# Bergvca/string_grouper

Hardware: AMD Instinct MI355X
Metric: hot-path rows/sec (the device path of match_strings: tokenise + tf-idf + postings + SpGEMM-topn, inputs resident in HBM), 663k-name self-join ntop=10 min_sim=0.8; match_strings end to end: match_strings_rows_per_s (higher is better)
Workload: dtype f32

## Files before the change

### string_grouper_amd/csrc/sg_internal.h

```cpp
#pragma once

#include <hip/hip_runtime.h>
#include <stdint.h>
#include <stdio.h>
#include <stdlib.h>
#include <string.h>

#include <map>
#include <memory>
#include <mutex>
#include <new>
#include <string>
#include <vector>

#include "../../include/sg_hip.h"

#define SG_WAVE 64
#define SG_NUM_XCD 8

void sg_set_error(const char *fmt, ...);

#define SG_HIP_TRY(expr)                                                                        \
    do {                                                                                        \
        hipError_t _e = (expr);                                                                 \
// ... 164 lines not shown
struct sg_csr {
    sg_ctx *ctx = nullptr;
    int64_t n_rows = 0, n_cols = 0, nnz = 0;
    int32_t dtype = SG_F32;
    const int64_t *d_indptr = nullptr;
    const int32_t *d_indices = nullptr;
    const void *d_data = nullptr;
    bool owned = false;
    mutable int props_state = 0;
    mutable float props_max_norm2 = 0.f;
    mutable uint32_t props_max_nnz = 0;
    bool from_vectoriser = false;
    mutable bool props_by_construction = false;
    mutable bool props_repeated_column = false;
    uint32_t *d_props_words = nullptr;
    double *d_row_norm = nullptr;
    mutable int left_state = 0;
    mutable struct SgCollapse *left_groups = nullptr;
    struct SgCollapse *rows_of = nullptr;
};

struct SgScoreCtx {
    const uint32_t *fwd_ptr = nullptr;
    const void *fwd = nullptr;
    const uint32_t *orig_of = nullptr;
    const void *blk = nullptr;
    uint32_t blk_bytes = 0;
    const uint4 *q8 = nullptr;
    float q8_scale = 0.f;
    uint32_t pad_ = 0;
};
#define SG_Q8_STRIDE 256u
#define SG_Q8_MAX_ENTRIES 60u

struct SgCollapse {
    sg_ctx *ctx = nullptr;
    int64_t n_orig = 0, n_u = 0;
    uint32_t *d_gid = nullptr;
    uint32_t *d_group_ptr = nullptr;
    uint32_t *d_members = nullptr;
    uint32_t *d_rep_rows = nullptr;
    int64_t *d_rep_start = nullptr;
    int32_t *d_rep_len = nullptr;
    struct sg_csr *unique = nullptr;
    const struct sg_csr *pending_src = nullptr;
};

struct sg_postings {
    sg_ctx *ctx = nullptr;
    int64_t n_right = 0, n_terms = 0, nnz = 0;
    int32_t dtype = SG_F32;
    int32_t tile_log2 = 12;
    int32_t n_tiles = 0;
    const int64_t *b_indptr = nullptr;
    const int32_t *b_indices = nullptr;
    const void *b_data = nullptr;
    uint32_t *d_seg = nullptr;
    uint32_t *d_term_len = nullptr;
    uint32_t *d_term_start = nullptr;
    int32_t *d_rows = nullptr;
    void *d_vals = nullptr;
    sg_csr src;
    int32_t split = 1;
    void *d_fwd = nullptr;
    uint32_t *d_fwd_ptr = nullptr;
    void *d_blk = nullptr;
    uint32_t blk_bytes = 0;
    void *d_q8 = nullptr;
    uint32_t *d_filt = nullptr;
    sg_csr *permuted = nullptr;
    uint32_t *d_orig_of = nullptr, *d_pos_of = nullptr;
    struct SgScoreCtx *d_score_ctx = nullptr;
    uint32_t *d_ends = nullptr;
    int32_t nt_pad = 0;
    int32_t fold_log2 = 0;
    uint32_t *d_ends8 = nullptr;
    int32_t nv_pad = 0;
    float norm_up = 0.f;
    uint32_t freq_min = 0;
    bool cosine_like = false;
    float max_norm2 = 0.f;
    SgCollapse *collapse = nullptr;
    const sg_csr *caller_b = nullptr;
    sg_csr caller_b_copy;
    int64_t n_right_caller = 0;
    mutable sg_postings *plain = nullptr;
    mutable sg_postings *exact_native = nullptr;
    mutable sg_postings *alt_tile = nullptr;
    sg_csr built_from;
    bool built_from_valid = false;
    bool tile_form = false;
    const sg_postings *view_of = nullptr;
    int32_t build_tile_cols = 0, build_flags = 0;
};

struct sg_topn {
    sg_ctx *ctx = nullptr;
    int64_t n_rows = 0, n_cols = 0;
    int32_t stride = 0;
    int32_t dtype = SG_F32;
    int32_t top_n_asked = 0;
// ... 6 lines not shown
    void operator()(sg_topn *r) const { sg_topn_free(r); }
};
using TopnPtr = std::unique_ptr<sg_topn, TopnFree>;
int topn_alloc(sg_ctx *ctx, int64_t n_rows, int64_t n_cols, int32_t stride, int32_t dtype, TopnPtr *out);
bool result_stride(int64_t n_rows, int64_t top_n, int64_t n_cols, int32_t *stride);
int result_overflow(int64_t n_rows, int32_t stride, const char *advice);
int sort_rows_by_column(sg_ctx *ctx, sg_topn *r);

struct sg_vocab {
    sg_ctx *ctx = nullptr;
    sg_vec_params params;
    int32_t bits_per_char = 7;
    int64_t n_terms = 0, n_docs = 0;
    int64_t key_space = 0;
    bool sorted_mode = false;
    int32_t *d_key_to_col = nullptr;
    uint64_t *d_keys = nullptr;
    int32_t *d_df = nullptr;
    void *d_idf = nullptr;
    bool idf_trusted = false;
    struct VocabImpl *impl = nullptr;
};

int sg_matchlist_device_view(const sg_matchlist *ml, int64_t *n_rows, int64_t *n_cols, int64_t *n_entries, int32_t *dtype,
                             const int64_t **row_ptr, const int32_t **cols, const void **vals);

#define SG_POSTINGS_NO_COLLAPSE (1 << 8)
#define SG_POSTINGS_TILE_FORM (1 << 11)
#define SG_POSTINGS_EXACT_ONLY (1 << 10)
int sg_csr_props(sg_ctx *ctx, const sg_csr *m, bool *cosine_like, float *max_norm2, uint32_t *max_nnz = nullptr);
bool sg_pruned_supports_tile(int32_t tile_log2);
int sg_postings_ensure_full(sg_ctx *ctx, const sg_postings *p);
bool sg_q8_applies(const sg_ctx *ctx, const sg_postings *Bt, double threshold);
int sg_spgemm_pruned_launch(sg_ctx *ctx, const sg_csr *A, const sg_postings *Bt, int32_t keep, sg_topn *r,
                            double threshold, double delta, uint32_t *row_counter,
                            uint32_t *flagged_count, uint32_t *flagged_rows, unsigned long long *stats);

int sg_spgemm_pruned_symmetric(sg_ctx *ctx, const sg_csr *A, const sg_postings *Bt, int32_t keep, sg_topn *r,
                               double threshold, double delta, unsigned long long *stats, bool *done, int64_t row_lo = 0,
                               int64_t row_hi = -1 , int32_t **export_pairs = nullptr,
                               int64_t *export_n = nullptr, int64_t row_step = 1 ,
                               bool exact_all = false );
int sg_selfjoin_merge_pairs(sg_ctx *ctx, sg_topn *r, const int32_t *d_pairs, int64_t n_pairs, int64_t row_lo, int64_t row_hi,
                            const uint32_t *pos_of ,
                            int64_t row_step = 1);

#define SG_PAIR_CHUNK 256u
#define SG_PAIR_NO_CHUNK 0xFFFFFFFFu
struct SgPairSink {
    uint32_t *d_i = nullptr;
    uint32_t *d_j = nullptr;
    void *d_s = nullptr;
    uint32_t *d_row_count = nullptr;
    uint32_t *d_chunk_count = nullptr;
    uint32_t *d_chunks_used = nullptr;
    unsigned long long *d_totals = nullptr;
    uint32_t chunks = 0;
};
unsigned sg_spgemm_exact_selfjoin_grid(const sg_ctx *ctx, const sg_postings *Bt = nullptr );
int sg_spgemm_exact_selfjoin_rows(sg_ctx *ctx, const sg_csr *A, const sg_postings *Bt, int32_t keep, sg_topn *r,
                                  double threshold, uint32_t *row_counter, const uint32_t *row_list,
                                  const uint32_t *row_list_len, const SgPairSink &sink, bool all_rows = false);

int sg_collapse_build(sg_ctx *ctx, const sg_csr *B, SgCollapse **out, bool left_side = false, bool defer_rows = false);
int sg_collapse_materialize(sg_ctx *ctx, SgCollapse *c);
int sg_csr_ensure_rows(sg_ctx *ctx, const sg_csr *m);
// ... 15 lines not shown
```

### string_grouper_amd/csrc/sg_postings.hip

```cpp
#include <stdlib.h>

#include <memory>
#include <optional>

#include "sg_internal.h"
#include "sg_scan.h"

__device__ __forceinline__ int64_t row_of_thread(int64_t g, int32_t tile_log2, int32_t n_tiles) {
    return ((g % n_tiles) << tile_log2) | (g / n_tiles);
}

template <typename T>
__global__ void __launch_bounds__(256) postings_count(const int64_t *__restrict__ indptr,
                                                      const int32_t *__restrict__ indices, int64_t n_rows,
                                                      int32_t tile_log2, int32_t n_tiles, uint32_t *seg_counts) {
    const int64_t j = row_of_thread((int64_t)blockIdx.x * blockDim.x + threadIdx.x, tile_log2, n_tiles);
    if (j >= n_rows) return;
    const int64_t lo = indptr[j], hi = indptr[j + 1];
    const uint32_t t = (uint32_t)(j >> tile_log2);
    for (int64_t p = lo; p < hi; ++p) {
        const int64_t bin = (int64_t)indices[p] * n_tiles + t;
        atomicAdd(&seg_counts[bin], 1u);
    }
}
// ... 625 lines not shown
    if (ends8)
        for (int32_t v = 0; v < nv_pad; ++v) {
            int64_t t = (int64_t)(v + 1) << fold_log2;
            if (t > n_tiles) t = n_tiles;
            ends8[k * nv_pad + v] = k == n_terms ? 0u : seg[k * n_tiles + t] << 2;
        }
}

__global__ void __launch_bounds__(256) null_postings_kernel(uint32_t *__restrict__ slack) {
    const uint32_t i = blockIdx.x * blockDim.x + threadIdx.x;
    slack[i] = sg_null_posting(i);
}

struct PermutedLenLoad {
    uint64_t n, minv, magic;
    const int32_t *len_of_row;
    const int64_t *indptr;
    uint32_t *pos_of, *orig_of;
    __device__ __forceinline__ int64_t operator()(int64_t p) const {
        const uint64_t x = (uint64_t)p * minv;
        const uint64_t q = __umul64hi(x, magic);
        int64_t rem = (int64_t)(x - q * n);
        if (rem < 0) rem += (int64_t)n;
        const uint32_t g = (uint32_t)rem;
        orig_of[p] = g;
        pos_of[g] = (uint32_t)p;
        return len_of_row ? (int64_t)len_of_row[g] : indptr[g + 1] - indptr[g];
    }
};

__device__ __forceinline__ uint32_t sg_q8_units(int64_t nnz) {
    return nnz > (int64_t)SG_Q8_MAX_ENTRIES ? 1u : (uint32_t)((nnz + 7) >> 2);
}
template <typename T>
__device__ __forceinline__ void q8_write_unit(uint4 *__restrict__ rec, uint32_t u, const int32_t *__restrict__ indices,
                                              const T *__restrict__ data, int64_t src, int64_t nnz, uint32_t first_packed,
                                              uint32_t name, float inv_norm) {
    auto entry = [&](int64_t e) -> uint32_t {
        if (e >= nnz) return 0u;
        const float q = ceilf((float)data[src + e] * inv_norm * 255.0f * 1.000002f);
        const uint32_t bq = q >= 255.0f ? 255u : (q >= 1.0f ? (uint32_t)q : 1u);
        return ((uint32_t)indices[src + e] << 8) | bq;
    };
    uint4 w;
    if (u == 0) {
        w = make_uint4(first_packed, name, (uint32_t)nnz | (nnz <= (int64_t)SG_Q8_MAX_ENTRIES ? 0u : 0x80000000u), 0u);
    } else {
        const int64_t e0 = 4 * (int64_t)u - 4;
        w = make_uint4(entry(e0), entry(e0 + 1), entry(e0 + 2), entry(e0 + 3));
    }
    rec[u] = w;
}

template <typename T>
__global__ void __launch_bounds__(256) q8_pack_kernel(const int64_t *__restrict__ indptr, const int32_t *__restrict__ indices,
                                                      const T *__restrict__ data, int64_t n_rows,
                                                      const uint32_t *__restrict__ orig_of ,
                                                      uint4 *__restrict__ q8, float inv_norm) {
    const int64_t p = ((int64_t)blockIdx.x * blockDim.x + threadIdx.x) >> 4;
    const uint32_t sub = threadIdx.x & 15;
    if (p >= n_rows) return;
    const int64_t base = indptr[0], src = indptr[p], n = indptr[p + 1] - src;
    if (sub < sg_q8_units(n))
        q8_write_unit<T>(q8 + p * (SG_Q8_STRIDE / 16), sub, indices, data, src, n, (uint32_t)(src - base),
                         orig_of ? orig_of[p] : (uint32_t)p, inv_norm);
}

#ifndef SG_GATHER_ROWS
#define SG_GATHER_ROWS 2
#endif
template <typename T>
__device__ __forceinline__ uint32_t q8_entry_of(int32_t k, T v, bool have, float inv_norm) {
    if (!have) return 0u;
    const float q = ceilf((float)v * inv_norm * 255.0f * 1.000002f);
    const uint32_t bq = q >= 255.0f ? 255u : (q >= 1.0f ? (uint32_t)q : 1u);
    return ((uint32_t)k << 8) | bq;
}
__device__ __forceinline__ void q8_write_round(uint4 *__restrict__ rec, int r, uint32_t wq, int sub, uint32_t units) {
    const int q = (sub - 4 * r - 1) & 3;
    const int base = (int)(threadIdx.x & 48u) + 4 * q;
    const uint32_t x0 = (uint32_t)__shfl((int)wq, base, 64), x1 = (uint32_t)__shfl((int)wq, base + 1, 64);
    const uint32_t x2 = (uint32_t)__shfl((int)wq, base + 2, 64), x3 = (uint32_t)__shfl((int)wq, base + 3, 64);
    if (sub >= 4 * r + 1 && sub <= 4 * r + 4 && (uint32_t)sub < units) rec[sub] = make_uint4(x0, x1, x2, x3);
}
template <typename T>
__device__ __forceinline__ void store_packed(void *__restrict__ fwd, int64_t at, int32_t k, T v) {
    if (sizeof(T) == 4) {
        reinterpret_cast<int2 *>(fwd)[at] = make_int2(k, __float_as_int((float)v));
    } else {
        const long long bits = __double_as_longlong((double)v);
        reinterpret_cast<int4 *>(fwd)[at] = make_int4(k, 0, (int)(bits & 0xffffffffll), (int)(bits >> 32));
    }
}
template <typename T>
__global__ void __launch_bounds__(256) gather_rows_kernel(const int64_t *__restrict__ indptr, const int32_t *__restrict__ indices,
                                                          const T *__restrict__ data, int64_t n_rows,
                                                          const uint32_t *__restrict__ orig_of,
                                                          const uint32_t *__restrict__ rep_rows ,
                                                          const int64_t *__restrict__ rep_start ,
                                                          const int32_t *__restrict__ rep_len,
                                                          const int64_t *__restrict__ perm_ptr, int32_t *__restrict__ perm_indices,
                                                          T *__restrict__ perm_data,
                                                          uint32_t *__restrict__ fwd_ptr , void *__restrict__ fwd,
                                                          uint4 *__restrict__ q8 , float inv_norm) {
    const int64_t grp = ((int64_t)blockIdx.x * blockDim.x + threadIdx.x) >> 4;
    const int sub = threadIdx.x & 15;
    const int64_t p0 = grp * SG_GATHER_ROWS;
    if (p0 > n_rows) return;
    bool valid[SG_GATHER_ROWS];
    uint32_t g[SG_GATHER_ROWS];
    int64_t src[SG_GATHER_ROWS], dst[SG_GATHER_ROWS];
    int32_t n[SG_GATHER_ROWS];
#pragma unroll
    for (int i = 0; i < SG_GATHER_ROWS; ++i) {
        valid[i] = p0 + i < n_rows;
        g[i] = valid[i] ? orig_of[p0 + i] : 0u;
        dst[i] = p0 + i <= n_rows ? perm_ptr[p0 + i] : 0;
    }
    if (rep_start) {
#pragma unroll
        for (int i = 0; i < SG_GATHER_ROWS; ++i) {
            src[i] = valid[i] ? rep_start[g[i]] : 0;
            n[i] = valid[i] ? rep_len[g[i]] : 0;
        }
    } else {
        int64_t j[SG_GATHER_ROWS];
#pragma unroll
        for (int i = 0; i < SG_GATHER_ROWS; ++i) j[i] = (valid[i] && rep_rows) ? (int64_t)rep_rows[g[i]] : (int64_t)g[i];
#pragma unroll
        for (int i = 0; i < SG_GATHER_ROWS; ++i) {
            src[i] = valid[i] ? indptr[j[i]] : 0;
            n[i] = valid[i] ? (int32_t)(indptr[j[i] + 1] - src[i]) : 0;
        }
    }
    int32_t k[SG_GATHER_ROWS][2];
    T v[SG_GATHER_ROWS][2];
#pragma unroll
    for (int i = 0; i < SG_GATHER_ROWS; ++i)
#pragma unroll
        for (int r = 0; r < 2; ++r) {
            const bool have = sub + 16 * r < n[i];
            k[i][r] = have ? indices[src[i] + sub + 16 * r] : 0;
            v[i][r] = have ? data[src[i] + sub + 16 * r] : (T)0;
        }
#pragma unroll
    for (int i = 0; i < SG_GATHER_ROWS; ++i) {
        const int64_t p = p0 + i;
        if (p == n_rows) {
            if (fwd_ptr && sub == 0) reinterpret_cast<uint2 *>(fwd_ptr)[p] = make_uint2((uint32_t)dst[i], 0u);
            if (fwd && sub < 8) store_packed<T>(fwd, dst[i] + sub, 0, (T)0);
        }
        if (!valid[i]) continue;
        const uint32_t units = q8 ? sg_q8_units(n[i]) : 0u;
        uint4 *rec = q8 ? q8 + p * (SG_Q8_STRIDE / 16) : nullptr;
        if (sub == 0) {
            if (fwd_ptr) reinterpret_cast<uint2 *>(fwd_ptr)[p] = make_uint2((uint32_t)dst[i], g[i]);
            if (q8) rec[0] = make_uint4((uint32_t)dst[i], g[i], (uint32_t)n[i] | (n[i] <= (int32_t)SG_Q8_MAX_ENTRIES ? 0u : 0x80000000u), 0u);
        }
#pragma unroll
        for (int r = 0; r < 2; ++r) {
            const int32_t e = sub + 16 * r;
            const bool have = e < n[i];
            if (have) {
                perm_indices[dst[i] + e] = k[i][r];
                perm_data[dst[i] + e] = v[i][r];
                if (fwd) store_packed<T>(fwd, dst[i] + e, k[i][r], v[i][r]);
            }
            if (units > 1u && 16 * r < n[i]) q8_write_round(rec, r, q8_entry_of<T>(k[i][r], v[i][r], have, inv_norm), sub, units);
        }
        for (int r = 2; 16 * r < n[i]; ++r) {
            const int32_t e = sub + 16 * r;
            const bool have = e < n[i];
            const int32_t kk = have ? indices[src[i] + e] : 0;
            const T vv = have ? data[src[i] + e] : (T)0;
            if (have) {
                perm_indices[dst[i] + e] = kk;
                perm_data[dst[i] + e] = vv;
                if (fwd) store_packed<T>(fwd, dst[i] + e, kk, vv);
            }
            if (units > 1u && r < 4) q8_write_round(rec, r, q8_entry_of<T>(kk, vv, have, inv_norm), sub, units);
        }
    }
}

__global__ void score_ctx_kernel(SgScoreCtx v, SgScoreCtx *out) {
    out[0] = v;
    v.q8 = nullptr;
    v.q8_scale = 0.f;
    out[1] = v;
}

struct PostingsFree {
    void operator()(sg_postings *p) const { sg_postings_free(p); }
};
using PostingsPtr = std::unique_ptr<sg_postings, PostingsFree>;

static sg_csr borrowed(const sg_csr &m) {
    sg_csr c = m;
    c.owned = false;
    c.d_props_words = nullptr;
    c.left_groups = nullptr;
    c.left_state = 0;
    return c;
}

static SgScoreCtx score_ctx_of(const sg_postings *p) {
    SgScoreCtx sc;
    if (!p->d_fwd_ptr) return sc;
    sc.fwd_ptr = p->d_fwd_ptr;
    sc.fwd = p->d_fwd;
    sc.blk = p->d_blk;
    sc.blk_bytes = p->blk_bytes;
    sc.orig_of = p->d_orig_of;
    sc.q8 = (const uint4 *)p->d_q8;
    sc.q8_scale = p->d_q8 ? __builtin_nextafterf((float)(255.0 / (double)p->norm_up * (1.0 - 1e-6)), 0.f) : 0.f;
    return sc;
}

static size_t lds_counter_bytes(int64_t n_cols) { return (size_t)n_cols * 4 + ((size_t)(n_cols + 31) / 32) * 4; }

struct BuildPlan {
    bool cosine_like = false;
    float max_norm2 = 0.f;
    int32_t tile_cols = 0, tile_log2 = 0;
    int64_t n_tiles = 0, n_bins = 0;
    bool want_pruned = false, will_filter = false, want_q8 = false, want_blk = false;
    bool permute = false;
    bool early_rows = false;
    bool lds_path = false, lazy_full = false;
    int32_t fold_log2 = 0, nt_pad = 0, nv_pad = 0;
    float norm_up = 0.f;
    uint32_t freq_min = 0;
    bool staged = false;
    int32_t chunk_rows = 0;
    uint32_t stage_cap = 0;
    uint32_t stage_alloc = 0;
    size_t staged_lds = 0;
    int32_t split = 1;
};

struct SplitCost {
    int32_t split = 1;
    int64_t parts = 0, part_rows = 0, chunks = 0, fill_rounds = 0;
    double fill_us = 0, table_us = 0, total_us = 0;
};
static constexpr double SG_SPLIT_US_PER_TERM_AND_CHUNK = 0.78e-3, SG_SPLIT_US_PER_POSTING = 2.9e-3, SG_SPLIT_US_PER_POSTING_RECOUNT = 0.53e-3,
                        SG_SPLIT_US_PER_CELL = 3.7e-6;
static constexpr int32_t SG_SPLIT_MAX = 16, SG_SPLIT_MIN_PART_ROWS = 512;
static SplitCost split_cost(int32_t split, int32_t tile_log2, int64_t n_tiles, int64_t n_terms, double mean_nnz, int32_t chunk_rows,
// ... 124 lines not shown
        pl.split = split;
    }
    *out = pl;
    return SG_OK;
}

struct EarlyRows {
    void *fwd = nullptr;
    uint32_t *fwd_ptr = nullptr;
    void *q8 = nullptr;
    bool written = false;
};

static int alloc_early_rows(Scratch &early, const sg_csr *B, const BuildPlan &plan, EarlyRows *rows) {
    if (!plan.early_rows) return SG_OK;
    SG_TRY(early.alloc_bytes(((size_t)B->nnz + 8) * (B->dtype == SG_F64 ? 16 : 8), &rows->fwd));
    SG_TRY(early.alloc(2 * ((size_t)B->n_rows + 2), &rows->fwd_ptr));
    if (plan.want_q8) SG_TRY(early.alloc_bytes((size_t)SG_Q8_STRIDE * ((size_t)B->n_rows + 1), &rows->q8));
    return SG_OK;
}

static uint64_t gcd_u64(uint64_t a, uint64_t b) {
    while (b) {
        const uint64_t t = a % b;
        a = b;
        b = t;
    }
    return a;
}

static int build_permuted(sg_ctx *ctx, const sg_csr *B, int64_t tile_cols, sg_postings *p,
                          SgCollapse *pending ,
                          EarlyRows *rows , float inv_norm) {
    if (ctx->opt_is("SG_PERMUTE", '0') || B->n_rows <= 2 * tile_cols || B->n_rows >= ((int64_t)1 << 31) || B->nnz <= 0) return SG_OK;
    const uint64_t n = (uint64_t)B->n_rows;
    uint64_t mult = (uint64_t)(0.6180339887498949 * (double)n) | 1ull;
    while (gcd_u64(mult, n) != 1) mult += 2;
    mult %= n;
    uint64_t minv = 0;
    {
        long long t0 = 0, t1 = 1, r0 = (long long)n, r1 = (long long)mult;
        while (r1 != 0) {
            const long long q = r0 / r1, t2 = t0 - q * t1, r2 = r0 - q * r1;
            t0 = t1;
            t1 = t2;
            r0 = r1;
            r1 = r2;
        }
        minv = (uint64_t)(t0 < 0 ? t0 + (long long)n : t0);
    }
    Scratch scratch(ctx);
    uint32_t *orig_of = nullptr, *pos_of = nullptr;
    int64_t *ptr = nullptr;
    int32_t *idx = nullptr;
    void *val = nullptr;
    const size_t vs = B->dtype == SG_F64 ? 8 : 4;
    const bool from_groups = pending && pending->pending_src;
    const bool by_group = from_groups && pending->d_rep_len != nullptr;
    SG_TRY(scratch.alloc((size_t)n + 1, &orig_of));
    SG_TRY(scratch.alloc((size_t)n + 1, &pos_of));
    SG_TRY(scratch.alloc((size_t)n + 2, &ptr));
    SG_TRY(scratch.alloc((size_t)B->nnz + 64, &idx));
    SG_TRY(scratch.alloc_bytes(((size_t)B->nnz + 64) * vs, &val));
    SG_TRY(sg_scan_launch<int64_t>(ctx, PermutedLenLoad{n, minv, (uint64_t)(~0ull / n) + 1ull, by_group ? pending->d_rep_len : (const int32_t *)nullptr, B->d_indptr, pos_of, orig_of},
                                   SgScanStoreArray<int64_t>{ptr}, (int64_t)n, ptr + n));
    const unsigned grid = (unsigned)((((n + 1 + SG_GATHER_ROWS - 1) / SG_GATHER_ROWS) * 16 + 255) / 256);
    const sg_csr *src = from_groups ? pending->pending_src : B;
    const uint32_t *rep_rows = from_groups ? pending->d_rep_rows : nullptr;
    const int64_t *rep_start = by_group ? pending->d_rep_start : nullptr;
    const int32_t *rep_len = by_group ? pending->d_rep_len : nullptr;
    by_dtype(B->dtype, [&](auto tag) {
        using T = decltype(tag);
        hipLaunchKernelGGL(gather_rows_kernel<T>, dim3(grid), dim3(256), 0, ctx->stream, src->d_indptr, src->d_indices,
                           (const T *)src->d_data, B->n_rows, (const uint32_t *)orig_of, rep_rows, rep_start, rep_len,
                           (const int64_t *)ptr, idx, (T *)val, rows->fwd_ptr, rows->fwd, (uint4 *)(rows->fwd_ptr ? rows->q8 : nullptr), inv_norm);
        return SG_OK;
    });
    if (hipGetLastError() != hipSuccess) return SG_ERR_HIP;
    sg_csr *m = new (std::nothrow) sg_csr();
    if (!m) return SG_ERR_OOM;
    rows->written = rows->fwd_ptr != nullptr;
    m->ctx = ctx;
    m->n_rows = B->n_rows;
    m->n_cols = B->n_cols;
    m->nnz = B->nnz;
    m->dtype = B->dtype;
    m->d_indptr = scratch.keep(ptr);
    m->d_indices = scratch.keep(idx);
    m->d_data = scratch.keep(val);
    m->owned = true;
    m->props_state = B->props_state;
    m->props_max_norm2 = B->props_max_norm2;
    m->props_max_nnz = B->props_max_nnz;
    m->props_repeated_column = B->props_repeated_column;
    p->permuted = m;
    p->d_orig_of = scratch.keep(orig_of);
    p->d_pos_of = scratch.keep(pos_of);
    return SG_OK;
}

static int row_block_bytes(sg_ctx *ctx, const sg_csr *B, uint32_t *out) {
    *out = 0;
    uint32_t max_nnz = 0;
    bool cl = false;
    float n2 = 0.f;
    if (B->props_max_nnz == 0 && !B->d_props_words) B->props_state = 0;
    SG_TRY(sg_csr_props(ctx, B, &cl, &n2, &max_nnz));
    const size_t es = B->dtype == SG_F64 ? 16 : 8;
// ... 2 lines not shown
        (ctx->total_mem == 0 || need * (size_t)B->n_rows < ctx->total_mem / 8))
        *out = (uint32_t)need;
    return SG_OK;
}

static int alloc_index(sg_ctx *ctx, sg_postings *p, const sg_csr *B_in, const sg_csr *B, const BuildPlan &plan, int32_t flags,
                       Scratch &early, EarlyRows *rows) {
    p->n_right = B->n_rows;
    p->n_terms = B->n_cols;
    p->nnz = B->nnz;
    p->dtype = B->dtype;
    p->tile_log2 = plan.tile_log2;
    p->tile_form = (flags & SG_POSTINGS_TILE_FORM) != 0;
    p->built_from = borrowed(*B_in);
    p->built_from_valid = true;
    p->n_tiles = (int32_t)plan.n_tiles;
    p->b_indptr = B_in->d_indptr;
    p->b_indices = B_in->d_indices;
    p->b_data = B_in->d_data;
    p->cosine_like = plan.cosine_like;
    p->max_norm2 = plan.max_norm2;
    p->src = borrowed(*B);
    p->split = plan.split;
    const size_t vs = 8;
    SG_TRY(sg_alloc(ctx, (size_t)plan.n_bins + 1, &p->d_seg));
    SG_TRY(sg_alloc(ctx, (size_t)B->n_cols + 1, &p->d_term_len));
    if (!plan.lazy_full && B->dtype == SG_F64) SG_TRY(sg_alloc(ctx, (size_t)B->nnz + 64, &p->d_rows));
    if (!plan.lazy_full) SG_TRY(ctx->alloc(((size_t)B->nnz + 64) * vs, &p->d_vals));
    if (!plan.will_filter) return SG_OK;
    if (plan.want_blk) {
        SG_TRY(row_block_bytes(ctx, B, &p->blk_bytes));
        if (p->blk_bytes) SG_TRY(ctx->alloc((size_t)p->blk_bytes * ((size_t)B->n_rows + 1), &p->d_blk));
    }
    if (rows->written) {
        p->d_fwd = early.keep(rows->fwd);
        p->d_fwd_ptr = early.keep(rows->fwd_ptr);
        p->d_q8 = early.keep(rows->q8);
    } else {
        if (!p->d_blk) SG_TRY(ctx->alloc(((size_t)B->nnz + 8) * (B->dtype == SG_F64 ? 16 : 8), &p->d_fwd));
        SG_TRY(sg_alloc(ctx, 2 * ((size_t)B->n_rows + 2), &p->d_fwd_ptr));
        if (plan.want_q8 && !p->d_blk) SG_TRY(ctx->alloc((size_t)SG_Q8_STRIDE * ((size_t)B->n_rows + 1), &p->d_q8));
    }
    SG_TRY(sg_alloc(ctx, (size_t)B->nnz + 512, &p->d_filt));
    p->nt_pad = plan.nt_pad;
    SG_TRY(sg_alloc(ctx, (size_t)(B->n_cols + 1) * (size_t)p->nt_pad + 4, &p->d_ends));
    p->fold_log2 = plan.fold_log2;
    p->nv_pad = plan.nv_pad;
    if (p->fold_log2 > 0) SG_TRY(sg_alloc(ctx, (size_t)(B->n_cols + 1) * (size_t)p->nv_pad + 4, &p->d_ends8));
    p->norm_up = plan.norm_up;
    p->freq_min = plan.freq_min;
    return SG_OK;
}

static int lds_count_scan_fill(sg_ctx *ctx, sg_postings *p, uint32_t *cnt ,
                               uint32_t *cnt16 ,
                               uint32_t *term_len, uint8_t *is_frequent, bool values_only, bool fill) {
    const sg_csr *B = &p->src;
    const int32_t split = p->split > 0 ? p->split : 1;
    const int64_t wgs64 = (int64_t)p->n_tiles * split;
    const unsigned wgs = (unsigned)wgs64;
    const size_t lds = lds_counter_bytes(B->n_cols);
    uint32_t *filt = values_only ? nullptr : p->d_filt;
    const float inv_norm = filt ? 1.0f / p->norm_up : 0.f;
    const int32_t fold_log2 = values_only ? 0 : p->fold_log2;
    SG_TRY(allow_dynamic_lds<postings_count_lds>(124 * 1024));
    hipLaunchKernelGGL(postings_count_lds, dim3(wgs), dim3(1024), (size_t)B->n_cols * 4, ctx->stream, B->d_indptr, B->d_indices,
// ... 87 lines not shown
        hipLaunchKernelGGL(ends_from_seg_kernel, dim3((unsigned)((p->n_terms + 256) / 256)), dim3(256), 0, ctx->stream,
                           (const uint32_t *)p->d_seg, p->n_terms, p->n_tiles, p->d_ends, p->nt_pad, p->d_ends8, p->nv_pad,
                           p->fold_log2);
    return hipGetLastError() == hipSuccess ? SG_OK : SG_ERR_HIP;
}

static int pack_rows(sg_ctx *ctx, sg_postings *p, bool rows_written) {
    const sg_csr *B = &p->src;
    if (p->d_fwd && !rows_written) {
        const size_t es = B->dtype == SG_F64 ? 16 : 8;
        if (hipMemsetAsync((char *)p->d_fwd + (size_t)B->nnz * es, 0, 8 * es, ctx->stream) != hipSuccess) return SG_ERR_HIP;
    }
    if (p->d_blk && B->n_rows > 0) {
        const int64_t work = B->n_rows * (int64_t)(p->blk_bytes / 16);
        const unsigned g3 = (unsigned)((work + 255) / 256);
        by_dtype(B->dtype, [&](auto tag) {
            using T = decltype(tag);
            hipLaunchKernelGGL(row_blocks_kernel<T>, dim3(g3), dim3(256), 0, ctx->stream, B->d_indptr, B->d_indices,
                               (const T *)B->d_data, B->n_rows, (const uint32_t *)p->d_orig_of, p->blk_bytes, p->d_blk);
            return SG_OK;
        });
        if (hipGetLastError() != hipSuccess) return SG_ERR_HIP;
    }
    if (p->d_fwd_ptr && !rows_written) {
        const int64_t work = B->nnz > B->n_rows + 1 ? B->nnz : B->n_rows + 1;
        const unsigned g2 = (unsigned)((work + 255) / 256);
        const unsigned g4 = (unsigned)((B->n_rows * 16 + 255) / 256);
        by_dtype(B->dtype, [&](auto tag) {
            using T = decltype(tag);
            hipLaunchKernelGGL(fwd_pack<T>, dim3(g2), dim3(256), 0, ctx->stream, B->d_indptr, B->d_indices,
                               (const T *)B->d_data, B->n_rows, B->nnz, (const uint32_t *)p->d_orig_of, p->d_fwd_ptr, p->d_fwd);
            if (p->d_q8 && B->n_rows > 0)
                hipLaunchKernelGGL(q8_pack_kernel<T>, dim3(g4), dim3(256), 0, ctx->stream, B->d_indptr, B->d_indices,
                                   (const T *)B->d_data, B->n_rows, (const uint32_t *)p->d_orig_of, (uint4 *)p->d_q8, 1.0f / p->norm_up);
            return SG_OK;
        });
        if (hipGetLastError() != hipSuccess) return SG_ERR_HIP;
    }
    return SG_OK;
}

static int write_aux(sg_ctx *ctx, sg_postings *p) {
    if (p->d_filt) {
        hipLaunchKernelGGL(null_postings_kernel, dim3(2), dim3(256), 0, ctx->stream, p->d_filt + p->nnz);
        if (hipGetLastError() != hipSuccess) return SG_ERR_HIP;
    }
    if (p->d_fwd_ptr) {
        SG_TRY(ctx->alloc(256, (void **)&p->d_score_ctx));
        hipLaunchKernelGGL(score_ctx_kernel, dim3(1), dim3(1), 0, ctx->stream, score_ctx_of(p), p->d_score_ctx);
        if (hipGetLastError() != hipSuccess) return SG_ERR_HIP;
    }
    return SG_OK;
}

static int build_index(sg_ctx *ctx, const sg_csr *B_in, int32_t tile_cols, int32_t flags, SgCollapse *pending,
                       std::optional<SgTimer> &timer, sg_postings **out) {
    bool cosine_like = false;
    float max_norm2 = 0.f;
    SG_TRY(sg_csr_props(ctx, B_in, &cosine_like, &max_norm2));
    SG_REQUIRE(!B_in->props_repeated_column,
               "the right-hand matrix has a row that names a column twice: the columns of a row must be distinct (sum the "
               "repeated entries first, e.g. scipy's sum_duplicates())");
    BuildPlan plan;
    SG_TRY(plan_build(ctx, B_in, tile_cols, flags, cosine_like, max_norm2, &plan));
    if (!timer) timer.emplace(ctx, SG_K_POSTINGS);
    PostingsPtr p(new (std::nothrow) sg_postings());
    if (!p) return SG_ERR_OOM;
// ... 114 lines not shown
```

### string_grouper_amd/csrc/sg_spgemm_pruned.hip

```cpp
#define SG_WATCH_NAME sg_debug_watch_pruned
#include "sg_k4_device.h"

#ifdef SG_DEBUG_WAVE_TIMES
__device__ unsigned long long sg_debug_wave_times[4 * 16384];
extern "C" int sg_debug_read_wave_times(unsigned long long *out, int clear) {
    if (hipMemcpyFromSymbol(out, HIP_SYMBOL(sg_debug_wave_times), sizeof(sg_debug_wave_times)) != hipSuccess) return 1;
    if (clear) {
        static unsigned long long zero[4 * 16384];
        if (hipMemcpyToSymbol(HIP_SYMBOL(sg_debug_wave_times), zero, sizeof(zero)) != hipSuccess) return 1;
    }
    return 0;
}
#endif

#ifndef SG_F64_STREAM_WAVES
#define SG_F64_STREAM_WAVES 4
#endif
#define SG_SCHED_FENCE() __builtin_amdgcn_sched_barrier(0)
#define SG_ROW_PARTS_LOG2 6
#define SG_ROW_PARTS 64u
#define SG_SURV_CAP 128

__device__ __forceinline__ uint64_t ballot64(bool p) { return __builtin_amdgcn_ballot_w64(p); }

// ... 157 lines not shown
        for (int q = 0; q < N; ++q) {
            const bool m1 = K[q].y == t[q], m2 = K[q].z == t[q], m3 = K[q].w == t[q];
            found[q] = K[q].x == t[q] || m1 || m2 || m3;
            bool walking = !found[q] && K[q].w != -1;
            h[q] += m1 ? 1u : (m2 ? 2u : (m3 ? 3u : 0u));
            if (__ballot(walking) != 0) {
                uint32_t g = (h[q] + 4u) & (SG_HASH_SLOTS - 1);
                int k = -1;
                SG_WD_DECL(wd_p);
                while (__ballot(walking) != 0) {
                    SG_WD(wd_p, SG_HASH_SLOTS + 2, 26)
                    if (walking) {
                        k = hk[g];
                        walking = k != t[q] && k != -1;
                        if (walking) g = (g + 1u) & (SG_HASH_SLOTS - 1);
                    }
                }
                asm volatile("" : "+v"(k), "+v"(g));
                if (!found[q] && K[q].w != -1) {
                    found[q] = k == t[q];
                    h[q] = g;
                }
            }
        }
    }
    T v[N];
#pragma unroll
    for (int q = 0; q < N; ++q) v[q] = ha[h[q]];
#pragma unroll
    for (int q = 0; q < N; ++q) out[q] = found[q] ? v[q] : (T)0;
}

template <typename T, bool WIDE>
__device__ __forceinline__ float q8_unit(uint4 w, const int *hk, const T *ha, int nnz, float ub) {
    const uint32_t e[4] = {w.x, w.y, w.z, w.w};
    if (WIDE) {
#pragma unroll
        for (int q = 0; q < 4; ++q)
            ub = __builtin_fmaf((float)row_value<T, true>(hk, ha, (int)(e[q] >> 8), nnz), (float)(e[q] & 255u), ub);
        return ub;
    }
    const int t[4] = {(int)(e[0] >> 8), (int)(e[1] >> 8), (int)(e[2] >> 8), (int)(e[3] >> 8)};
    T a[4];
    row_values<T, 4>(hk, ha, t, a);
#pragma unroll
    for (int q = 0; q < 4; ++q) ub = __builtin_fmaf((float)a[q], (float)(e[q] & 255u), ub);
    return ub;
}

template <typename T, bool WIDE>
__device__ __forceinline__ bool q8_passes(int j, const int *hk, const T *ha, int nnz, const uint4 *__restrict__ q8, float bar,
                                          uint32_t &pb, uint32_t &pe, int &row_of_j) {
    const bool have = j >= 0;
    const size_t rec = (size_t)(have ? j : 0) * (SG_Q8_STRIDE / 16u);
    uint4 cur = make_uint4(0u, 0u, 0x80000000u, 0u), nxt = make_uint4(0u, 0u, 0u, 0u);
    if (have) {
        cur = load_global_u4(q8, rec);
        nxt = load_global_u4(q8, rec + 1);
    }
    const uint32_t n_j = cur.z & 0x7fffffffu;
    const bool whole = (cur.z >> 31) == 0u;
    pb = cur.x;
    pe = cur.x + n_j;
    row_of_j = have ? (int)cur.y : j;
    const uint32_t units = whole ? (n_j + 7u) >> 2 : 1u;
    float ub = 0.f;
    SG_WD_DECL(wd_q);
    for (uint32_t u = 1u;; ++u) {
        SG_WD(wd_q, 20, 25)
        if (__ballot(u < units) == 0) break;
        cur = nxt;
        if (u + 1u < units) nxt = load_global_u4(q8, rec + u + 1u);
        if (u < units) ub = q8_unit<T, WIDE>(cur, hk, ha, nnz, ub);
    }
    return have && (!whole || ub >= bar);
}

template <typename T, bool WIDE>
__device__ __forceinline__ T exact_score_blocks(int j, const int *hk, const T *ha, int nnz, const SgScoreCtx *__restrict__ sc,
                                                int &row_of_j) {
    constexpr int ES = sizeof(T) == 4 ? 8 : 16;
    constexpr int EPU = 32 / ES;
    T sum = (T)0;
    row_of_j = j;
    const bool have = j >= 0;
    const uint4 *base = reinterpret_cast<const uint4 *>(reinterpret_cast<const char *>(sc->blk) +
                                                        (size_t)(have ? j : 0) * (size_t)sc->blk_bytes);
    uint4 U[2];
#pragma unroll
    for (int e = 0; e < 2; ++e) U[e] = make_uint4(0u, 0u, 0u, 0u);
    if (have) {
#pragma unroll
        for (int e = 0; e < 2; ++e) U[e] = base[e];
    }
    const int nnz_j = have ? (int)U[0].y : -1;
    if (have) row_of_j = (int)U[0].x;
    uint32_t touched = 0;
    auto use = [&](int idx, uint32_t term, T val) {
        const bool valid = idx >= 1 && idx <= nnz_j;
        T a = (T)0;
        if (valid) a = row_value<T, WIDE>(hk, ha, (int)term, nnz);
        sum = add_rn<T>(sum, mul_rn<T>(a, valid ? val : (T)0));
    };
    SG_WD_DECL(wd_b);
    for (int u = 0;; ++u) {
        SG_WD(wd_b, 64, 24)
// ... 1325 lines not shown
    uint32_t *row_counter = nullptr;
    uint32_t *flagged_count = nullptr, *flagged_rows = nullptr;
    const PairList *pl = nullptr;
};

struct PrunedLaunch {
    uint32_t *row_counter;
    uint32_t *out_count, *out_rows;
    const uint32_t *in_rows = nullptr, *in_len = nullptr;
    uint32_t *heavy_count = nullptr, *heavy_rows = nullptr;
    uint32_t part_cfg = 0;
};

struct RowList {
    uint32_t *base = nullptr;
    uint32_t *count() const { return base; }
    uint32_t *counter() const { return base ? base + 1 : nullptr; }
    uint32_t *rows() const { return base ? base + 4 : nullptr; }
};

template <typename T, int TILE_LOG2, bool SYM, bool WIDE, int FOLD_LOG2>
static int launch_pruned(const PrunedJob &job, const PrunedLaunch &l) {
    sg_ctx *ctx = job.ctx;
    const sg_csr *A = job.A;
    const sg_postings *Bt = job.Bt;
    const sg_topn *r = job.r;
    const PairList &pl = *job.pl;
    const T thr = (T)job.threshold;
    const size_t lds = pruned_lds(TILE_LOG2, FOLD_LOG2, A->dtype);
    unsigned grid = pruned_grid(ctx, TILE_LOG2, SYM ? (int64_t)pl.rows() : A->n_rows, FOLD_LOG2, A->dtype);
    if (WIDE && grid > (unsigned)ctx->num_cu * 4u && (double)A->nnz <= 48.0 * (double)A->n_rows) grid = (unsigned)ctx->num_cu * 4u;
    constexpr bool SPLITS = SYM && !WIDE && FOLD_LOG2 > 0;
    const bool share = SPLITS && (l.heavy_count != nullptr || l.part_cfg != 0u);
    auto kernel = share ? spgemm_topn_pruned_kernel<T, TILE_LOG2, SYM, WIDE, FOLD_LOG2, SPLITS>
                        : spgemm_topn_pruned_kernel<T, TILE_LOG2, SYM, WIDE, FOLD_LOG2, false>;
    hipLaunchKernelGGL(kernel, dim3(grid), dim3(64), lds, ctx->stream, A->d_indptr,
                       A->d_indices, (const T *)A->d_data, (uint32_t)A->n_rows, (const uint32_t *)Bt->d_seg,
                       (const uint32_t *)Bt->d_ends, Bt->nt_pad, (uint32_t)Bt->n_terms,
                       (const uint32_t *)Bt->d_filt, Bt->n_tiles,
                       (const SgScoreCtx *)Bt->d_score_ctx + (sg_q8_applies(ctx, Bt, (double)thr) ? 0 : 1), job.keep, r->stride, thr,
                       job.s_budget, Bt->norm_up, Bt->freq_min, r->d_cols,
                       (T *)r->d_vals,
                       r->d_counts, l.row_counter, l.out_count, l.out_rows, job.stats, pl.d_sink, pl.sink.chunks, pl.row_lo, pl.row_hi,
                       l.in_rows, l.in_len, (const uint32_t *)Bt->d_ends8, Bt->nv_pad, (uint32_t)(Bt->nnz * 4), (uint32_t)Bt->n_right,
                       l.heavy_count, l.heavy_rows, pl.row_step, ctx->opt_is("SG_DEAL", 'f') ? 1u : 0u, l.part_cfg);
    SG_HIP_TRY(hipGetLastError());
    return SG_OK;
}

static uint32_t heavy_part_cfg(const sg_ctx *ctx, const sg_csr *A, const PairList &range, int32_t tile_log2, int32_t fold_log2) {
    uint32_t heavy_rounds = 0;
    if ((range.row_lo > 0 || (int64_t)range.row_hi < A->n_rows || range.row_step > 1) && 2 * (int64_t)range.rows() < A->n_rows) {
        const double n_idx = (double)A->n_rows;
        const double rows_per_wave = (double)range.rows() / (double)pruned_grid(ctx, tile_log2, (int64_t)range.rows(), fold_log2, A->dtype);
        const double rounds_per_row = 2.0 * 7.2e-5 * n_idx * (0.5 * ((double)range.row_lo + (double)range.row_hi) / n_idx);
        const double share = ctx->opt_double("SG_HEAVY_SHARE", 0.0);
        const double bar_share = share > 0.0 ? share : 0.05;
        const double bar = bar_share * rows_per_wave * rounds_per_row;
        heavy_rounds = bar < 128.0 ? 128u : (bar > 1.0e9 ? 1000000000u : (uint32_t)bar);
    }
    heavy_rounds = (uint32_t)ctx->opt_int("SG_HEAVY_ROUNDS", (int)heavy_rounds) & 0x7fffffffu;
    if (heavy_rounds > 0x0fffffffu) heavy_rounds = 0x0fffffffu;
    uint32_t handover_shift = heavy_rounds >= 512u ? 1u : (heavy_rounds >= 256u ? 2u : 3u);
    handover_shift = (uint32_t)ctx->opt_int("SG_HANDOVER_SHIFT", (int)handover_shift) & 7u;
    if (heavy_rounds) heavy_rounds |= handover_shift << 28;
    return heavy_rounds;
// ... 342 lines not shown
```

Before: 109.1 million.

## Add early-exit Cauchy-Schwarz bound to q8 candidate upper-bound scoring

Stores per-row remainder norms (ceil sqrt of quantized squared-sum of the entries past several unit checkpoints) in the previously unused fourth word of each q8 record header. While accumulating the quantized upper bound, the scorer estimates the query's unmatched norm and stops reading further units once ub plus the Cauchy-Schwarz bound on the rest falls below the threshold. This is meant to cut global loads and gather work for candidates that are clearly rejected. The cost is extra packing work, a per-candidate wave reduction of the query norm, and a resync kernel when the option is toggled.

After: 111.0 million, median of 6. 1.02x the previous value.

```diff
diff --git a/string_grouper_amd/csrc/sg_internal.h b/string_grouper_amd/csrc/sg_internal.h
--- a/string_grouper_amd/csrc/sg_internal.h
+++ b/string_grouper_amd/csrc/sg_internal.h
@@ -220,6 +220,8 @@
 };
 #define SG_Q8_STRIDE 256u
 #define SG_Q8_MAX_ENTRIES 60u
+#define SG_Q8_REST_UNIT(f) ((f) == 0 ? 2u : (f) == 1 ? 3u : (f) == 2 ? 4u : 6u)
+#define SG_Q8_REST_UNKNOWN 255u
 
 struct SgCollapse {
     sg_ctx *ctx = nullptr;
@@ -255,6 +257,7 @@
     void *d_blk = nullptr;
     uint32_t blk_bytes = 0;
     void *d_q8 = nullptr;
+    mutable bool q8_early = true;
     uint32_t *d_filt = nullptr;
     sg_csr *permuted = nullptr;
     uint32_t *d_orig_of = nullptr, *d_pos_of = nullptr;
@@ -327,6 +330,7 @@
 bool sg_pruned_supports_tile(int32_t tile_log2);
 int sg_postings_ensure_full(sg_ctx *ctx, const sg_postings *p);
 bool sg_q8_applies(const sg_ctx *ctx, const sg_postings *Bt, double threshold);
+int sg_postings_sync_q8_early(sg_ctx *ctx, const sg_postings *Bt);
 int sg_spgemm_pruned_launch(sg_ctx *ctx, const sg_csr *A, const sg_postings *Bt, int32_t keep, sg_topn *r,
                             double threshold, double delta, uint32_t *row_counter,
                             uint32_t *flagged_count, uint32_t *flagged_rows, unsigned long long *stats);
diff --git a/string_grouper_amd/csrc/sg_postings.hip b/string_grouper_amd/csrc/sg_postings.hip
--- a/string_grouper_amd/csrc/sg_postings.hip
+++ b/string_grouper_amd/csrc/sg_postings.hip
@@ -681,10 +681,19 @@
 __device__ __forceinline__ uint32_t sg_q8_units(int64_t nnz) {
     return nnz > (int64_t)SG_Q8_MAX_ENTRIES ? 1u : (uint32_t)((nnz + 7) >> 2);
 }
+__device__ __forceinline__ uint32_t q8_root_up(uint32_t s) {
+    uint32_t r = (uint32_t)sqrtf((float)s);
+    while (r * r < s) ++r;
+    while (r > 0u && (r - 1u) * (r - 1u) >= s) --r;
+    return r < SG_Q8_REST_UNKNOWN ? r : SG_Q8_REST_UNKNOWN;
+}
+__device__ __forceinline__ uint32_t q8_rest_word(const uint32_t (&sums)[4], uint32_t unknown) {
+    return unknown | q8_root_up(sums[0]) | (q8_root_up(sums[1]) << 8) | (q8_root_up(sums[2]) << 16) | (q8_root_up(sums[3]) << 24);
+}
 template <typename T>
 __device__ __forceinline__ void q8_write_unit(uint4 *__restrict__ rec, uint32_t u, const int32_t *__restrict__ indices,
                                               const T *__restrict__ data, int64_t src, int64_t nnz, uint32_t first_packed,
-                                              uint32_t name, float inv_norm) {
+                                              uint32_t name, float inv_norm, uint32_t rest_unknown) {
     auto entry = [&](int64_t e) -> uint32_t {
         if (e >= nnz) return 0u;
         const float q = ceilf((float)data[src + e] * inv_norm * 255.0f * 1.000002f);
@@ -693,7 +702,15 @@
     };
     uint4 w;
     if (u == 0) {
-        w = make_uint4(first_packed, name, (uint32_t)nnz | (nnz <= (int64_t)SG_Q8_MAX_ENTRIES ? 0u : 0x80000000u), 0u);
+        const bool whole = nnz <= (int64_t)SG_Q8_MAX_ENTRIES;
+        uint32_t sums[4] = {0u, 0u, 0u, 0u};
+        for (int64_t e = 4 * (int64_t)SG_Q8_REST_UNIT(0); whole && e < nnz; ++e) {
+            const uint32_t bq = entry(e) & 255u;
+#pragma unroll
+            for (int f = 0; f < 4; ++f)
+                if (e >= 4 * (int64_t)SG_Q8_REST_UNIT(f)) sums[f] += bq * bq;
+        }
+        w = make_uint4(first_packed, name, (uint32_t)nnz | (whole ? 0u : 0x80000000u), q8_rest_word(sums, whole ? rest_unknown : ~0u));
     } else {
         const int64_t e0 = 4 * (int64_t)u - 4;
         w = make_uint4(entry(e0), entry(e0 + 1), entry(e0 + 2), entry(e0 + 3));
@@ -705,14 +722,14 @@
 __global__ void __launch_bounds__(256) q8_pack_kernel(const int64_t *__restrict__ indptr, const int32_t *__restrict__ indices,
                                                       const T *__restrict__ data, int64_t n_rows,
                                                       const uint32_t *__restrict__ orig_of ,
-                                                      uint4 *__restrict__ q8, float inv_norm) {
+                                                      uint4 *__restrict__ q8, float inv_norm, uint32_t rest_unknown) {
     const int64_t p = ((int64_t)blockIdx.x * blockDim.x + threadIdx.x) >> 4;
     const uint32_t sub = threadIdx.x & 15;
     if (p >= n_rows) return;
     const int64_t base = indptr[0], src = indptr[p], n = indptr[p + 1] - src;
     if (sub < sg_q8_units(n))
         q8_write_unit<T>(q8 + p * (SG_Q8_STRIDE / 16), sub, indices, data, src, n, (uint32_t)(src - base),
-                         orig_of ? orig_of[p] : (uint32_t)p, inv_norm);
+                         orig_of ? orig_of[p] : (uint32_t)p, inv_norm, rest_unknown);
 }
 
 #ifndef SG_GATHER_ROWS
@@ -751,7 +768,8 @@
                                                           const int64_t *__restrict__ perm_ptr, int32_t *__restrict__ perm_indices,
                                                           T *__restrict__ perm_data,
                                                           uint32_t *__restrict__ fwd_ptr , void *__restrict__ fwd,
-                                                          uint4 *__restrict__ q8 , float inv_norm) {
+                                                          uint4 *__restrict__ q8 , float inv_norm,
+                                                          uint32_t rest_unknown ) {
     const int64_t grp = ((int64_t)blockIdx.x * blockDim.x + threadIdx.x) >> 4;
     const int sub = threadIdx.x & 15;
     const int64_t p0 = grp * SG_GATHER_ROWS;
@@ -802,10 +820,14 @@
         if (!valid[i]) continue;
         const uint32_t units = q8 ? sg_q8_units(n[i]) : 0u;
         uint4 *rec = q8 ? q8 + p * (SG_Q8_STRIDE / 16) : nullptr;
-        if (sub == 0) {
-            if (fwd_ptr) reinterpret_cast<uint2 *>(fwd_ptr)[p] = make_uint2((uint32_t)dst[i], g[i]);
-            if (q8) rec[0] = make_uint4((uint32_t)dst[i], g[i], (uint32_t)n[i] | (n[i] <= (int32_t)SG_Q8_MAX_ENTRIES ? 0u : 0x80000000u), 0u);
-        }
+        if (sub == 0 && fwd_ptr) reinterpret_cast<uint2 *>(fwd_ptr)[p] = make_uint2((uint32_t)dst[i], g[i]);
+        uint32_t rest[4] = {0u, 0u, 0u, 0u};
+        auto add_rest = [&](uint32_t wq, int32_t e) {
+            const uint32_t bq = wq & 255u;
+#pragma unroll
+            for (int f = 0; f < 4; ++f)
+                if (e >= 4 * (int32_t)SG_Q8_REST_UNIT(f)) rest[f] += bq * bq;
+        };
 #pragma unroll
         for (int r = 0; r < 2; ++r) {
             const int32_t e = sub + 16 * r;
@@ -815,7 +837,11 @@
                 perm_data[dst[i] + e] = v[i][r];
                 if (fwd) store_packed<T>(fwd, dst[i] + e, k[i][r], v[i][r]);
             }
-            if (units > 1u && 16 * r < n[i]) q8_write_round(rec, r, q8_entry_of<T>(k[i][r], v[i][r], have, inv_norm), sub, units);
+            if (units > 1u && 16 * r < n[i]) {
+                const uint32_t wq = q8_entry_of<T>(k[i][r], v[i][r], have, inv_norm);
+                add_rest(wq, e);
+                q8_write_round(rec, r, wq, sub, units);
+            }
         }
         for (int r = 2; 16 * r < n[i]; ++r) {
             const int32_t e = sub + 16 * r;
@@ -827,9 +853,41 @@
                 perm_data[dst[i] + e] = vv;
                 if (fwd) store_packed<T>(fwd, dst[i] + e, kk, vv);
             }
-            if (units > 1u && r < 4) q8_write_round(rec, r, q8_entry_of<T>(kk, vv, have, inv_norm), sub, units);
-        }
-    }
+            if (units > 1u && r < 4) {
+                const uint32_t wq = q8_entry_of<T>(kk, vv, have, inv_norm);
+                add_rest(wq, e);
+                q8_write_round(rec, r, wq, sub, units);
+            }
+        }
+        if (q8) {
+            const bool whole = n[i] <= (int32_t)SG_Q8_MAX_ENTRIES;
+            if (units > 1u) {
+#pragma unroll
+                for (int f = 0; f < 4; ++f)
+#pragma unroll
+                    for (int d = 1; d < 16; d <<= 1) rest[f] += (uint32_t)__shfl_xor((int)rest[f], d, 64);
+            }
+            if (sub == 0)
+                rec[0] = make_uint4((uint32_t)dst[i], g[i], (uint32_t)n[i] | (whole ? 0u : 0x80000000u),
+                                    q8_rest_word(rest, whole ? rest_unknown : ~0u));
+        }
+    }
+}
+
+__global__ void __launch_bounds__(256) q8_rest_kernel(uint4 *__restrict__ q8, int64_t n_rows, uint32_t rest_unknown) {
+    const int64_t p = (int64_t)blockIdx.x * blockDim.x + threadIdx.x;
+    if (p >= n_rows) return;
+    uint32_t *rec = reinterpret_cast<uint32_t *>(q8 + p * (SG_Q8_STRIDE / 16));
+    const uint32_t word2 = rec[2], n = word2 & 0x7fffffffu;
+    const bool whole = (word2 >> 31) == 0u && n <= SG_Q8_MAX_ENTRIES;
+    uint32_t sums[4] = {0u, 0u, 0u, 0u};
+    for (uint32_t e = 4u * SG_Q8_REST_UNIT(0); whole && rest_unknown == 0u && e < n; ++e) {
+        const uint32_t bq = rec[4u + e] & 255u;
+#pragma unroll
+        for (int f = 0; f < 4; ++f)
+            if (e >= 4u * SG_Q8_REST_UNIT(f)) sums[f] += bq * bq;
+    }
+    rec[3] = q8_rest_word(sums, whole ? rest_unknown : ~0u);
 }
 
 __global__ void score_ctx_kernel(SgScoreCtx v, SgScoreCtx *out) {
@@ -864,6 +922,17 @@
     sc.q8 = (const uint4 *)p->d_q8;
     sc.q8_scale = p->d_q8 ? __builtin_nextafterf((float)(255.0 / (double)p->norm_up * (1.0 - 1e-6)), 0.f) : 0.f;
     return sc;
+}
+
+static uint32_t q8_rest_unknown(const sg_ctx *ctx) { return ctx->opt_is("SG_Q8_EARLY", '0') ? ~0u : 0u; }
+int sg_postings_sync_q8_early(sg_ctx *ctx, const sg_postings *Bt) {
+    const bool want = q8_rest_unknown(ctx) == 0u;
+    if (!Bt->d_q8 || Bt->q8_early == want || Bt->n_right <= 0) return SG_OK;
+    hipLaunchKernelGGL(q8_rest_kernel, dim3((unsigned)((Bt->n_right + 255) / 256)), dim3(256), 0, ctx->stream, (uint4 *)Bt->d_q8,
+                       Bt->n_right, want ? 0u : ~0u);
+    if (hipGetLastError() != hipSuccess) return SG_ERR_HIP;
+    Bt->q8_early = want;
+    return SG_OK;
 }
 
 static size_t lds_counter_bytes(int64_t n_cols) { return (size_t)n_cols * 4 + ((size_t)(n_cols + 31) / 32) * 4; }
@@ -1054,6 +1123,7 @@
 static int build_permuted(sg_ctx *ctx, const sg_csr *B, int64_t tile_cols, sg_postings *p,
                           SgCollapse *pending ,
                           EarlyRows *rows , float inv_norm) {
+    const uint32_t rest_unknown = q8_rest_unknown(ctx);
     if (ctx->opt_is("SG_PERMUTE", '0') || B->n_rows <= 2 * tile_cols || B->n_rows >= ((int64_t)1 << 31) || B->nnz <= 0) return SG_OK;
     const uint64_t n = (uint64_t)B->n_rows;
     uint64_t mult = (uint64_t)(0.6180339887498949 * (double)n) | 1ull;
@@ -1095,7 +1165,8 @@
         using T = decltype(tag);
         hipLaunchKernelGGL(gather_rows_kernel<T>, dim3(grid), dim3(256), 0, ctx->stream, src->d_indptr, src->d_indices,
                            (const T *)src->d_data, B->n_rows, (const uint32_t *)orig_of, rep_rows, rep_start, rep_len,
-                           (const int64_t *)ptr, idx, (T *)val, rows->fwd_ptr, rows->fwd, (uint4 *)(rows->fwd_ptr ? rows->q8 : nullptr), inv_norm);
+                           (const int64_t *)ptr, idx, (T *)val, rows->fwd_ptr, rows->fwd, (uint4 *)(rows->fwd_ptr ? rows->q8 : nullptr), inv_norm,
+                           rest_unknown);
         return SG_OK;
     });
     if (hipGetLastError() != hipSuccess) return SG_ERR_HIP;
@@ -1164,6 +1235,7 @@
         SG_TRY(row_block_bytes(ctx, B, &p->blk_bytes));
         if (p->blk_bytes) SG_TRY(ctx->alloc((size_t)p->blk_bytes * ((size_t)B->n_rows + 1), &p->d_blk));
     }
+    p->q8_early = q8_rest_unknown(ctx) == 0u;
     if (rows->written) {
         p->d_fwd = early.keep(rows->fwd);
         p->d_fwd_ptr = early.keep(rows->fwd_ptr);
@@ -1317,7 +1389,8 @@
                                (const T *)B->d_data, B->n_rows, B->nnz, (const uint32_t *)p->d_orig_of, p->d_fwd_ptr, p->d_fwd);
             if (p->d_q8 && B->n_rows > 0)
                 hipLaunchKernelGGL(q8_pack_kernel<T>, dim3(g4), dim3(256), 0, ctx->stream, B->d_indptr, B->d_indices,
-                                   (const T *)B->d_data, B->n_rows, (const uint32_t *)p->d_orig_of, (uint4 *)p->d_q8, 1.0f / p->norm_up);
+                                   (const T *)B->d_data, B->n_rows, (const uint32_t *)p->d_orig_of, (uint4 *)p->d_q8, 1.0f / p->norm_up,
+                                   q8_rest_unknown(ctx));
             return SG_OK;
         });
         if (hipGetLastError() != hipSuccess) return SG_ERR_HIP;
diff --git a/string_grouper_amd/csrc/sg_spgemm_pruned.hip b/string_grouper_amd/csrc/sg_spgemm_pruned.hip
--- a/string_grouper_amd/csrc/sg_spgemm_pruned.hip
+++ b/string_grouper_amd/csrc/sg_spgemm_pruned.hip
@@ -213,12 +213,15 @@
 }
 
 template <typename T, bool WIDE>
-__device__ __forceinline__ float q8_unit(uint4 w, const int *hk, const T *ha, int nnz, float ub) {
+__device__ __forceinline__ float q8_unit(uint4 w, const int *hk, const T *ha, int nnz, float ub, float &matched) {
     const uint32_t e[4] = {w.x, w.y, w.z, w.w};
     if (WIDE) {
 #pragma unroll
-        for (int q = 0; q < 4; ++q)
-            ub = __builtin_fmaf((float)row_value<T, true>(hk, ha, (int)(e[q] >> 8), nnz), (float)(e[q] & 255u), ub);
+        for (int q = 0; q < 4; ++q) {
+            const float a = (float)row_value<T, true>(hk, ha, (int)(e[q] >> 8), nnz);
+            ub = __builtin_fmaf(a, (float)(e[q] & 255u), ub);
+            matched = __builtin_fmaf(a, a, matched);
+        }
         return ub;
     }
     const int t[4] = {(int)(e[0] >> 8), (int)(e[1] >> 8), (int)(e[2] >> 8), (int)(e[3] >> 8)};
@@ -226,7 +229,33 @@
     row_values<T, 4>(hk, ha, t, a);
 #pragma unroll
     for (int q = 0; q < 4; ++q) ub = __builtin_fmaf((float)a[q], (float)(e[q] & 255u), ub);
+#pragma unroll
+    for (int q = 0; q < 4; ++q) matched = __builtin_fmaf((float)a[q], (float)a[q], matched);
     return ub;
+}
+
+__device__ __forceinline__ float wave_sum(float v) {
+#define SG_DPP_F32(x, ctrl) __int_as_float(__builtin_amdgcn_update_dpp(0, __float_as_int(x), ctrl, 0xf, 0xf, true))
+    v += SG_DPP_F32(v, 0xB1);
+    v += SG_DPP_F32(v, 0x4E);
+    v += SG_DPP_F32(v, 0x141);
+    v += SG_DPP_F32(v, 0x140);
+#undef SG_DPP_F32
+    return (wave_read<float>(v, 0) + wave_read<float>(v, 16)) + (wave_read<float>(v, 32) + wave_read<float>(v, 48));
+}
+
+template <typename T, bool WIDE>
+__device__ __forceinline__ float staged_row_norm2_up(const int *hk, const T *ha, int nnz) {
+    const int lane = threadIdx.x;
+    float s = 0.f;
+#pragma unroll
+    for (int h = 0; h < 2; ++h) {
+        const int at = lane + 64 * h;
+        const bool holds = WIDE ? at < nnz : hk[at] != -1;
+        const float a = holds ? (float)ha[at] : 0.f;
+        s = __builtin_fmaf(a, a, s);
+    }
+    return wave_sum(s) * 1.00002f;
 }
 
 template <typename T, bool WIDE>
@@ -239,20 +268,29 @@
         cur = load_global_u4(q8, rec);
         nxt = load_global_u4(q8, rec + 1);
     }
+    const float na2_up = staged_row_norm2_up<T, WIDE>(hk, ha, nnz);
+    const float bar_lo = __int_as_float(__builtin_amdgcn_readfirstlane(__float_as_int(bar * 0.99998f)));
     const uint32_t n_j = cur.z & 0x7fffffffu;
     const bool whole = (cur.z >> 31) == 0u;
+    const uint32_t rest = cur.w;
     pb = cur.x;
     pe = cur.x + n_j;
     row_of_j = have ? (int)cur.y : j;
-    const uint32_t units = whole ? (n_j + 7u) >> 2 : 1u;
-    float ub = 0.f;
+    uint32_t units = whole ? (n_j + 7u) >> 2 : 1u;
+    float ub = 0.f, matched = 0.f;
     SG_WD_DECL(wd_q);
     for (uint32_t u = 1u;; ++u) {
         SG_WD(wd_q, 20, 25)
         if (__ballot(u < units) == 0) break;
         cur = nxt;
         if (u + 1u < units) nxt = load_global_u4(q8, rec + u + 1u);
-        if (u < units) ub = q8_unit<T, WIDE>(cur, hk, ha, nnz, ub);
+        if (u < units) ub = q8_unit<T, WIDE>(cur, hk, ha, nnz, ub, matched);
+        const int f = u == SG_Q8_REST_UNIT(0) ? 0 : u == SG_Q8_REST_UNIT(1) ? 8 : u == SG_Q8_REST_UNIT(2) ? 16 : u == SG_Q8_REST_UNIT(3) ? 24 : -1;
+        if (f >= 0) {
+            const uint32_t r8 = (rest >> f) & 255u;
+            const float a_rest = __builtin_amdgcn_sqrtf(fmaxf(na2_up - matched, 1e-30f));
+            if (u + 1u < units && r8 != SG_Q8_REST_UNKNOWN && __builtin_fmaf(a_rest, (float)r8, ub) < bar_lo) units = u + 1u;
+        }
     }
     return have && (!whole || ub >= bar);
 }
@@ -1644,6 +1682,7 @@
     if (WIDE && grid > (unsigned)ctx->num_cu * 4u && (double)A->nnz <= 48.0 * (double)A->n_rows) grid = (unsigned)ctx->num_cu * 4u;
     constexpr bool SPLITS = SYM && !WIDE && FOLD_LOG2 > 0;
     const bool share = SPLITS && (l.heavy_count != nullptr || l.part_cfg != 0u);
+    if (sg_q8_applies(ctx, Bt, (double)thr)) SG_TRY(sg_postings_sync_q8_early(ctx, Bt));
     auto kernel = share ? spgemm_topn_pruned_kernel<T, TILE_LOG2, SYM, WIDE, FOLD_LOG2, SPLITS>
                         : spgemm_topn_pruned_kernel<T, TILE_LOG2, SYM, WIDE, FOLD_LOG2, false>;
     hipLaunchKernelGGL(kernel, dim3(grid), dim3(64), lds, ctx->stream, A->d_indptr,
```
